# libxsmm/libxsmm

Measured on NVIDIA H100. Metric: batched BRGEMM GFLOP/s (bf16, m=n=k=64, br=8, batch=65536/GPU, unique operands), higher is better.
Workload: dtype bf16

## Files before the change

### libxsmm_b200/csrc/gemm_tc.cu

```cuda
#include <cuda.h>
#include <cuda_runtime.h>
#include <stdint.h>
#include <stdio.h>
#include <stdlib.h>
#include <string.h>
#include "xb_internal.h"
#include "xb_device.cuh"
#include "xb_tma.cuh"
#include "xb_wgmma.cuh"
#include "xb_epilogue.cuh"

namespace {

enum { XB_WG_SS16 = 0, XB_WG_RS16 = 1, XB_WG_RS8 = 2 };

struct WgParams {
  int m, n, k;
  int kchunks, kc_elems, kinst;
  int stages, stage_bytes, a_bytes, tx_bytes;
  int bf16;
  int sgn;
  unsigned long long br;
  long long count;
  char* c; long long tile_stride_c, ldc;
  int ep_mode, c_esz, beta0;
  float scf;
  const int4* sets; char* const* cptrs; int pair;
};

template <int NC>
__device__ __forceinline__ void wg_mma16(int bf16, float (&d)[NC / 2], uint64_t a, uint64_t b, int scale_d) {
  if (NC == 16) { if (bf16) xb_wgmma_ss_bf16_n16<1>(*reinterpret_cast<float(*)[8]>(&d), a, b, scale_d); else xb_wgmma_ss_f16_n16<1>(*reinterpret_cast<float(*)[8]>(&d), a, b, scale_d); }
  if (NC == 32) { if (bf16) xb_wgmma_ss_bf16_n32<1>(*reinterpret_cast<float(*)[16]>(&d), a, b, scale_d); else xb_wgmma_ss_f16_n32<1>(*reinterpret_cast<float(*)[16]>(&d), a, b, scale_d); }
  if (NC == 64) { if (bf16) xb_wgmma_ss_bf16_n64<1>(*reinterpret_cast<float(*)[32]>(&d), a, b, scale_d); else xb_wgmma_ss_f16_n64<1>(*reinterpret_cast<float(*)[32]>(&d), a, b, scale_d); }
}
template <int NC>
__device__ __forceinline__ void wg_mma16_rs(int bf16, float (&d)[NC / 2], const uint32_t (&a)[4], uint64_t b, int scale_d) {
  if (NC == 16) { if (bf16) xb_wgmma_rs_bf16_n16(*reinterpret_cast<float(*)[8]>(&d), a, b, scale_d); else xb_wgmma_rs_f16_n16(*reinterpret_cast<float(*)[8]>(&d), a, b, scale_d); }
  if (NC == 32) { if (bf16) xb_wgmma_rs_bf16_n32(*reinterpret_cast<float(*)[16]>(&d), a, b, scale_d); else xb_wgmma_rs_f16_n32(*reinterpret_cast<float(*)[16]>(&d), a, b, scale_d); }
  if (NC == 64) { if (bf16) xb_wgmma_rs_bf16_n64(*reinterpret_cast<float(*)[32]>(&d), a, b, scale_d); else xb_wgmma_rs_f16_n64(*reinterpret_cast<float(*)[32]>(&d), a, b, scale_d); }
}
#define XB_WG_I8(N) \
  switch (sgn) { case 0: xb_wgmma_rs_u8u8_n##N(*reinterpret_cast<int(*)[N / 2]>(&d), a, b, scale_d); break; \
                 case 1: xb_wgmma_rs_u8s8_n##N(*reinterpret_cast<int(*)[N / 2]>(&d), a, b, scale_d); break; \
                 case 2: xb_wgmma_rs_s8u8_n##N(*reinterpret_cast<int(*)[N / 2]>(&d), a, b, scale_d); break; \
                 default: xb_wgmma_rs_s8s8_n##N(*reinterpret_cast<int(*)[N / 2]>(&d), a, b, scale_d); break; }
template <int NC>
__device__ __forceinline__ void wg_mma8_rs(int sgn, float (&d)[NC / 2], const uint32_t (&a)[4], uint64_t b, int scale_d) {
  if (NC == 16) { XB_WG_I8(16) }
  if (NC == 32) { XB_WG_I8(32) }
  if (NC == 64) { XB_WG_I8(64) }
}
#undef XB_WG_I8

template <int AMODE, int NC, int NCH, int WG>
__global__ void __launch_bounds__(WG * 128 + 32, (NCH == 1 && WG == 1) ? 3 : 1)
gemm_wg_kernel(const __grid_constant__ CUtensorMap map_a, const __grid_constant__ CUtensorMap map_b, const WgParams P) {
  extern __shared__ uint8_t smem_raw[];
  uint8_t* smem = (uint8_t*)(((uintptr_t)smem_raw + 1023) & ~(uintptr_t)1023);
  const uint32_t smem_base = xb_smem_u32(smem);
  const int S = P.stages;
  const uint32_t full0 = xb_smem_u32(smem + (size_t)S * P.stage_bytes), empty0 = full0 + 8 * S;
  const int warp = threadIdx.x >> 5, lane = threadIdx.x & 31;
  const long long G = gridDim.x, b = blockIdx.x;
  const long long n_local = (b < P.count) ? (P.count - b + G - 1) / G : 0;
  const bool pooled = P.sets != nullptr;

  if (threadIdx.x == 0) {
    asm volatile("prefetch.tensormap [%0];" :: "l"(&map_a) : "memory");
    asm volatile("prefetch.tensormap [%0];" :: "l"(&map_b) : "memory");
    for (int i = 0; i < S; ++i) { xb_mbar_init(full0 + 8 * i, 1); xb_mbar_init(empty0 + 8 * i, 4 * WG); }
    asm volatile("fence.mbarrier_init.release.cluster;" ::: "memory");
  }
  __syncthreads();

  if (warp == 4 * WG) {
    if (lane == 0) {
      int stage = 0; uint32_t phase = 0;
      for (long long i = 0; i < n_local; ++i) {
        const long long t = b + i * G;
        int ta0 = (int)t, ta1 = (int)t, tb = (int)t, m1 = 64;
        if (pooled) {
          const int4 st = P.sets[t];
          ta0 = st.x; ta1 = P.pair ? st.y : st.x; tb = st.z; m1 = P.pair ? 0 : 64;
        }
        for (unsigned long long r = 0; r < P.br; ++r) {
          for (int kc = 0; kc < P.kchunks; ++kc) {
            xb_mbar_wait(empty0 + 8 * stage, phase ^ 1);
            const uint32_t full = full0 + 8 * stage, sa = smem_base + stage * P.stage_bytes, sb = sa + P.a_bytes;
            xb_mbar_expect_tx(full, (uint32_t)P.tx_bytes);
            if (AMODE == XB_WG_SS16) {
              xb_tma_load_4d(sa, &map_a, full, 0, kc * 64, (int)r, ta0);
              if (WG == 2) xb_tma_load_4d(sa + 8192, &map_a, full, m1, kc * 64, (int)r, ta1);
            } else {
              xb_tma_load_4d(sa, &map_a, full, 0, kc * 32, (int)r, ta0);
            }
            xb_tma_load_4d(sb, &map_b, full, kc * P.kc_elems, 0, (int)r, tb);
            if (++stage == S) { stage = 0; phase ^= 1; }
          }
        }
      }
    }
    return;
  }

  const int g = warp >> 2, wq = warp & 3;
  const int row_a = 64 * g + 16 * wq + (lane >> 2), q = lane & 3;
  const int loads = (int)P.br * P.kchunks;
  float acc[NCH][NC / 2];
  int stage = 0; uint32_t phase = 0;
  for (long long i = 0; i < n_local; ++i) {
    const long long t = b + i * G;
    int kc = 0, prev = -1;
    for (int l = 0; l < loads; ++l) {
      xb_mbar_wait(full0 + 8 * stage, phase);
      const uint32_t sa = smem_base + stage * P.stage_bytes, sb = sa + P.a_bytes;
      const int krem = P.k - kc * P.kc_elems;
      const int ksteps = (krem >= P.kc_elems) ? P.kc_elems / P.kinst : (krem + P.kinst - 1) / P.kinst;
      xb_wgmma_fence();
      for (int ks = 0; ks < ksteps; ++ks) {
        const int scale_d = (l > 0 || ks > 0) ? 1 : 0;
        if (AMODE == XB_WG_SS16) {
          const uint64_t ad = xb_wg_desc(sa + 8192u * g + 2048u * ks, 8192, 1024, 1);
#pragma unroll
          for (int c = 0; c < NCH; ++c) wg_mma16<NC>(P.bf16, acc[c], ad, xb_wg_desc(sb + (uint32_t)(c * NC * 128) + 32u * ks, 16, 1024, 1), scale_d);
        } else {
          const uint32_t* w = reinterpret_cast<const uint32_t*>(smem + (size_t)stage * P.stage_bytes);
          uint32_t a[4];
#pragma unroll
          for (int j = 0; j < 4; ++j) {
            const int rr = row_a + 8 * (j & 1), kw = 8 * ks + q + 4 * (j >> 1);
            a[j] = (rr < P.m) ? w[kw * P.m + rr] : 0u;
          }
#pragma unroll
          for (int c = 0; c < NCH; ++c) {
            const uint64_t bd = xb_wg_desc(sb + (uint32_t)(c * NC * 128) + 32u * ks, 16, 1024, 1);
            if (AMODE == XB_WG_RS16) wg_mma16_rs<NC>(P.bf16, acc[c], a, bd, scale_d);
            else wg_mma8_rs<NC>(P.sgn, acc[c], a, bd, scale_d);
          }
        }
      }
      xb_wgmma_commit();
      xb_wgmma_wait<1>();
      if (prev >= 0) { __syncwarp(); if (lane == 0) xb_mbar_arrive(empty0 + 8 * prev); }
      prev = stage;
      if (++kc == P.kchunks) kc = 0;
      if (++stage == S) { stage = 0; phase ^= 1; }
    }
    xb_wgmma_wait<0>();
    if (prev >= 0) { __syncwarp(); if (lane == 0) xb_mbar_arrive(empty0 + 8 * prev); }
    char* ctile; int row0 = 64 * g;
    if (!pooled) ctile = P.c + t * P.tile_stride_c;
    else if (P.pair) { ctile = P.cptrs[2 * t + g]; row0 = 0; }
    else ctile = P.cptrs[t];
    if (ctile == nullptr) continue;
    char* cbase = ctile - (long long)(64 * g - row0) * P.c_esz;
#pragma unroll
    for (int c = 0; c < NCH; ++c) {
      if (c * NC >= P.n) break;
      xb_ep_store_frag<NC / 2>(P.ep_mode, P.beta0, *reinterpret_cast<const uint32_t(*)[NC / 2]>(&acc[c]), cbase, 64 * g, c * NC,
                               P.m + (64 * g - row0), P.n, P.ldc * P.c_esz, P.c_esz, P.scf);
    }
  }
}

int g_num_sms = 0;

int env_int(const char* name, int fallback) {
  const char* e = getenv(name);
  return (e != nullptr && *e != 0) ? atoi(e) : fallback;
}

int num_sms() {
  if (g_num_sms == 0) {
    int dev = 0; cudaGetDevice(&dev);
    cudaDeviceGetAttribute(&g_num_sms, cudaDevAttrMultiProcessorCount, dev);
    if (g_num_sms <= 0) g_num_sms = 132;
  }
  return g_num_sms;
}

template <int AMODE, int NC, int NCH, int WG>
cudaError_t launch_one(long long grid, size_t smem, cudaStream_t stream, const CUtensorMap& ma, const CUtensorMap& mb, const WgParams& P) {
  static unsigned long long done = 0ull;
  if (xb_rt_first_use_on_device(&done)) cudaFuncSetAttribute(gemm_wg_kernel<AMODE, NC, NCH, WG>, cudaFuncAttributeMaxDynamicSharedMemorySize, 227 * 1024);
  gemm_wg_kernel<AMODE, NC, NCH, WG><<<(unsigned int)grid, WG * 128 + 32, smem, stream>>>(ma, mb, P);
  return cudaGetLastError();
}

template <int AMODE, int WG>
cudaError_t launch_n(int nt, long long grid, size_t smem, cudaStream_t stream, const CUtensorMap& ma, const CUtensorMap& mb, const WgParams& P) {
  switch (nt) {
    case 16:  return launch_one<AMODE, 16, 1, WG>(grid, smem, stream, ma, mb, P);
    case 32:  return launch_one<AMODE, 32, 1, WG>(grid, smem, stream, ma, mb, P);
    case 64:  return launch_one<AMODE, 64, 1, WG>(grid, smem, stream, ma, mb, P);
    case 128: return launch_one<AMODE, 64, 2, WG>(grid, smem, stream, ma, mb, P);
    default:  return launch_one<AMODE, 64, 4, WG>(grid, smem, stream, ma, mb, P);
  }
}

int n_tile(int n) { return n <= 16 ? 16 : (n <= 32 ? 32 : (n <= 64 ? 64 : (n <= 128 ? 128 : 256))); }

void plan_stages(WgParams& P, int nt, int wg, int* ctas) {
  int c = (nt == 64 && wg == 1) || nt < 64 ? 3 : 1;
  while (c > 1 && 2 * P.stage_bytes + 2048 > (227 * 1024) / c) --c;
  int st = ((227 * 1024) / c - 2048) / P.stage_bytes; if (st > 8) st = 8; if (st < 2) st = 2;
  P.stages = st; *ctas = c;
}

int wg_launch(int amode, int wg, int nt, const WgParams& P, int ctas, const CUtensorMap& ma, const CUtensorMap& mb, const char* where) {
  const size_t smem = (size_t)P.stages * P.stage_bytes + 1024  + 2 * 8 * P.stages;
  long long grid = P.count; if (grid > (long long)num_sms() * ctas) grid = (long long)num_sms() * ctas; if (grid < 1) grid = 1;
  cudaStream_t stream = (cudaStream_t)xb_rt_stream();
  cudaError_t e;
  if (amode == XB_WG_SS16) e = (wg == 2) ? launch_n<XB_WG_SS16, 2>(nt, grid, smem, stream, ma, mb, P) : launch_n<XB_WG_SS16, 1>(nt, grid, smem, stream, ma, mb, P);
  else if (amode == XB_WG_RS16) e = (wg == 2) ? launch_n<XB_WG_RS16, 2>(nt, grid, smem, stream, ma, mb, P) : launch_n<XB_WG_RS16, 1>(nt, grid, smem, stream, ma, mb, P);
  else e = (wg == 2) ? launch_n<XB_WG_RS8, 2>(nt, grid, smem, stream, ma, mb, P) : launch_n<XB_WG_RS8, 1>(nt, grid, smem, stream, ma, mb, P);
  xb_rt_count_launch();
  if (e != cudaSuccess) { xb_rt_note_error((int)e, where); return (int)e; }
  return 0;
}

}

extern "C" int xb_gemm_tc_supported(const xb_gemm_desc* d);
extern "C" int xb_gemm_tc_shape_ok(const xb_gemm_desc* d) {
  xb_gemm_desc t = *d;
  t.br_type = 0;
  return xb_gemm_tc_supported(&t);
}

extern "C" int xb_gemm_tc_supported(const xb_gemm_desc* d) {
  const unsigned int bad = LIBXSMM_GEMM_FLAG_TRANS_A | LIBXSMM_GEMM_FLAG_TRANS_B | LIBXSMM_GEMM_FLAG_VNNI_A
                         | LIBXSMM_GEMM_FLAG_VNNI_B | LIBXSMM_GEMM_FLAG_VNNI_C | LIBXSMM_GEMM_FLAG_DECOMPRESS_A_VIA_BITMASK;
  if ((d->flags & bad) != 0) return 0;
  if (!(d->ta == d->tb && (d->ta == LIBXSMM_DATATYPE_BF16 || d->ta == LIBXSMM_DATATYPE_F16))) return 0;
  if (d->tcomp != LIBXSMM_DATATYPE_F32) return 0;
  if (d->ta == LIBXSMM_DATATYPE_BF16 && !(d->tc == LIBXSMM_DATATYPE_F32 || d->tc == LIBXSMM_DATATYPE_BF16)) return 0;
  if (d->ta == LIBXSMM_DATATYPE_F16 && !(d->tc == LIBXSMM_DATATYPE_F32 || d->tc == LIBXSMM_DATATYPE_F16)) return 0;
  if (d->m < 16 || d->n < 16 || d->k < 16 || d->m > 128 || d->n > 256 || d->k > 4096) return 0;
  if ((d->lda % 8) != 0 || (d->ldb % 8) != 0) return 0;
  if (!(d->br_type == 0 || d->br_type == 3)) return 0;
  if (d->br_type == 3 && ((d->br_stride_a % 16) != 0 || (d->br_stride_b % 16) != 0 || d->br_stride_a <= 0 || d->br_stride_b <= 0)) return 0;
  return 1;
}

static int tc_launch_common(const xb_gemm_launch* L, const xb_tc_pool* pool);
extern "C" int xb_gemm_tc_launch(const xb_gemm_launch* L) { return tc_launch_common(L, nullptr); }
extern "C" int xb_gemm_tc_launch_pooled(const xb_gemm_desc* d, const xb_tc_pool* pool, unsigned long long br, long long count) {
  xb_gemm_launch L; memset(&L, 0, sizeof(L));
  L.d = *d; L.count = count; L.br = br;
  L.a = pool->base_a; L.b = pool->base_b; L.c = (void*)pool->cptrs;
  L.tile_stride_a = pool->set_a; L.tile_stride_b = pool->set_b; L.tile_stride_c = 16;
  return tc_launch_common(&L, pool);
}

static int tc_launch_common(const xb_gemm_launch* L, const xb_tc_pool* pool) {
  const xb_gemm_desc& d = L->d;
  const char* a = (const char*)L->a; const char* b = (const char*)L->b; char* c = (char*)L->c;
  long long sa = L->tile_stride_a, sb = L->tile_stride_b, sc = L->tile_stride_c;
  unsigned long long br = L->br;
  if (L->recs != nullptr) return xb_gemm_simt_launch(L);
  if (a == nullptr && c == nullptr) { a = (const char*)L->one.a; b = (const char*)L->one.b; c = (char*)L->one.c; br = L->one.br; sa = sb = sc = 0; }
  if (d.br_type == 0 && pool == nullptr) br = 1;
  const int es = 2;
  const bool aligned = (((uintptr_t)a | (uintptr_t)b) & 15) == 0 && (sa % 16) == 0 && (sb % 16) == 0
                    && (L->count == 1 || (sa > 0 && sb > 0));
  xb_encode_tiled_fn enc = xb_tma_encoder();
  if (br == 0 || !aligned || L->count <= 0 || br > 0x7fffffffull || L->count > 0x7fffffffll || enc == nullptr) {
    return (pool != nullptr) ? 1 : xb_gemm_simt_launch(L);
  }

  const int wg = (d.m <= 64 && !(pool != nullptr && pool->pair)) ? 1 : 2;
  const int nt = n_tile(d.n);
  WgParams P; memset(&P, 0, sizeof(P));
  P.m = d.m; P.n = d.n; P.k = d.k;
  P.kc_elems = 64; P.kinst = 16; P.kchunks = (d.k + 63) / 64;
  P.a_bytes = wg * 8192; P.stage_bytes = P.a_bytes + nt * 128; P.tx_bytes = P.stage_bytes;
  P.bf16 = (d.ta == LIBXSMM_DATATYPE_BF16) ? 1 : 0;
  P.br = br; P.count = L->count; P.c = c; P.tile_stride_c = sc; P.ldc = d.ldc;
  if (pool != nullptr) { P.sets = (const int4*)pool->sets; P.cptrs = (char* const*)pool->cptrs; P.pair = pool->pair; }
  P.beta0 = (d.flags & LIBXSMM_GEMM_FLAG_BETA_0) ? 1 : 0;
  P.ep_mode = xb_ep_mode(d.ta, d.tc, &P.c_esz);
  int ctas = 1;
  plan_stages(P, nt, wg, &ctas);

  const CUtensorMapDataType dt = P.bf16 ? CU_TENSOR_MAP_DATA_TYPE_BFLOAT16 : CU_TENSOR_MAP_DATA_TYPE_FLOAT16;
  const cuuint32_t estr[4] = {1, 1, 1, 1};
  const size_t ext_a = ((size_t)(d.k - 1) * d.lda + d.m) * es, ext_b = ((size_t)(d.n - 1) * d.ldb + d.k) * es;
  const cuuint64_t pad_a = (ext_a + 15) & ~(size_t)15, pad_b = (ext_b + 15) & ~(size_t)15;
  CUtensorMap map_a, map_b;
  {
    const cuuint64_t dims[4] = {(cuuint64_t)d.m, (cuuint64_t)d.k, (cuuint64_t)br, (cuuint64_t)(pool ? pool->nsets_a : L->count)};
    const cuuint64_t strides[3] = {(cuuint64_t)d.lda * es, pool ? (cuuint64_t)pool->blk_a : ((d.br_type == 3) ? (cuuint64_t)d.br_stride_a : pad_a),
                                   pool ? (cuuint64_t)pool->set_a : ((L->count > 1) ? (cuuint64_t)sa : pad_a)};
    const cuuint32_t box[4] = {64, 64, 1, 1};
    if (CUDA_SUCCESS != enc(&map_a, dt, 4, (void*)a, dims, strides, box, estr, CU_TENSOR_MAP_INTERLEAVE_NONE,
                            CU_TENSOR_MAP_SWIZZLE_128B, CU_TENSOR_MAP_L2_PROMOTION_L2_256B, CU_TENSOR_MAP_FLOAT_OOB_FILL_NONE))
      return (pool != nullptr) ? 1 : xb_gemm_simt_launch(L);
  }
  {
    const cuuint64_t dims[4] = {(cuuint64_t)d.k, (cuuint64_t)d.n, (cuuint64_t)br, (cuuint64_t)(pool ? pool->nsets_b : L->count)};
    const cuuint64_t strides[3] = {(cuuint64_t)d.ldb * es, pool ? (cuuint64_t)pool->blk_b : ((d.br_type == 3) ? (cuuint64_t)d.br_stride_b : pad_b),
                                   pool ? (cuuint64_t)pool->set_b : ((L->count > 1) ? (cuuint64_t)sb : pad_b)};
    const cuuint32_t box[4] = {64, (cuuint32_t)nt, 1, 1};
    if (CUDA_SUCCESS != enc(&map_b, dt, 4, (void*)b, dims, strides, box, estr, CU_TENSOR_MAP_INTERLEAVE_NONE,
                            CU_TENSOR_MAP_SWIZZLE_128B, CU_TENSOR_MAP_L2_PROMOTION_L2_256B, CU_TENSOR_MAP_FLOAT_OOB_FILL_NONE))
      return (pool != nullptr) ? 1 : xb_gemm_simt_launch(L);
  }
  return wg_launch(XB_WG_SS16, wg, nt, P, ctas, map_a, map_b, "gemm_tc");
}

extern "C" int xb_gemm_ts_supported(const xb_gemm_desc* d) {
  const unsigned int bad = LIBXSMM_GEMM_FLAG_TRANS_A | LIBXSMM_GEMM_FLAG_TRANS_B | LIBXSMM_GEMM_FLAG_VNNI_B | LIBXSMM_GEMM_FLAG_VNNI_C
                         | LIBXSMM_GEMM_FLAG_DECOMPRESS_A_VIA_BITMASK | LIBXSMM_GEMM_FLAG_INTLV_A_FORMAT;
  const int a8 = (d->ta == LIBXSMM_DATATYPE_I8 || d->ta == LIBXSMM_DATATYPE_U8), b8 = (d->tb == LIBXSMM_DATATYPE_I8 || d->tb == LIBXSMM_DATATYPE_U8);
  static int enabled = -1;
  if (enabled < 0) enabled = env_int("LIBXSMM_B200_TS", 1) != 0 ? 1 : 0;
  if (!enabled || (d->flags & bad) != 0 || d->fuse_colbias != 0 || d->cp_op != 0) return 0;
  if (a8 && b8) {
    if (d->tcomp != LIBXSMM_DATATYPE_I32 || !(d->tc == LIBXSMM_DATATYPE_I32 || d->tc == LIBXSMM_DATATYPE_F32)) return 0;
    if ((d->flags & LIBXSMM_GEMM_FLAG_VNNI_A) == 0 && d->tc != LIBXSMM_DATATYPE_F32) return 0;
    if ((d->k % 4) != 0 || (d->ldb % 16) != 0) return 0;
  } else if (d->ta == d->tb && (d->ta == LIBXSMM_DATATYPE_BF16 || d->ta == LIBXSMM_DATATYPE_F16)) {
    if ((d->flags & LIBXSMM_GEMM_FLAG_VNNI_A) == 0 || d->tcomp != LIBXSMM_DATATYPE_F32) return 0;
    if (d->ta == LIBXSMM_DATATYPE_BF16 && !(d->tc == LIBXSMM_DATATYPE_F32 || d->tc == LIBXSMM_DATATYPE_BF16)) return 0;
    if (d->ta == LIBXSMM_DATATYPE_F16 && !(d->tc == LIBXSMM_DATATYPE_F32 || d->tc == LIBXSMM_DATATYPE_F16)) return 0;
    if ((d->k % 2) != 0 || (d->ldb % 8) != 0) return 0;
  } else return 0;
  if (d->m < 4 || d->m > 128 || (d->m % 4) != 0 || (d->lda % 4) != 0 || d->n < 1 || d->n > 128 || d->k > 8192) return 0;
  if (!(d->br_type == 0 || d->br_type == 3)) return 0;
  if (d->br_type == 3 && ((d->br_stride_a % 16) != 0 || (d->br_stride_b % 16) != 0 || d->br_stride_a <= 0 || d->br_stride_b <= 0)) return 0;
  return 1;
}

extern "C" int xb_gemm_ts_launch(const xb_gemm_launch* L) {
  const xb_gemm_desc& d = L->d;
  const char* a = (const char*)L->a; const char* b = (const char*)L->b; char* c = (char*)L->c;
  long long sa = L->tile_stride_a, sb = L->tile_stride_b, sc = L->tile_stride_c;
  unsigned long long br = L->br;
  if (L->recs != nullptr) return xb_gemm_simt_launch(L);
  if (a == nullptr && c == nullptr) { a = (const char*)L->one.a; b = (const char*)L->one.b; c = (char*)L->one.c; br = L->one.br; sa = sb = sc = 0; }
  if (d.br_type == 0) br = 1;
  const bool aligned = (((uintptr_t)a | (uintptr_t)b) & 15) == 0 && (sa % 16) == 0 && (sb % 16) == 0 && (L->count == 1 || (sa > 0 && sb > 0));
  xb_encode_tiled_fn enc = xb_tma_encoder();
  if (br == 0 || !aligned || L->count <= 0 || br > 0x7fffffffull || L->count > 0x7fffffffll || enc == nullptr) return xb_gemm_simt_launch(L);

  const int is_i8 = (d.ta == LIBXSMM_DATATYPE_I8 || d.ta == LIBXSMM_DATATYPE_U8);
  const int v = is_i8 ? 4 : 2, es = is_i8 ? 1 : 2;
  const int wg = (d.m <= 64) ? 1 : 2, nt = n_tile(d.n);
  WgParams P; memset(&P, 0, sizeof(P));
  P.m = d.m; P.n = d.n; P.k = d.k;
  P.kc_elems = 128 / es; P.kinst = is_i8 ? 32 : 16; P.kchunks = (d.k + P.kc_elems - 1) / P.kc_elems;
  P.a_bytes = (d.m * 128 + 1023) & ~1023;
  P.stage_bytes = P.a_bytes + nt * 128; P.tx_bytes = d.m * 128 + nt * 128;
  P.bf16 = (d.ta == LIBXSMM_DATATYPE_BF16) ? 1 : 0;
  P.sgn = ((d.ta == LIBXSMM_DATATYPE_I8) ? 2 : 0) | ((d.tb == LIBXSMM_DATATYPE_I8) ? 1 : 0);
  P.br = br; P.count = L->count; P.c = c; P.tile_stride_c = sc; P.ldc = d.ldc;
  P.beta0 = (d.flags & LIBXSMM_GEMM_FLAG_BETA_0) ? 1 : 0; P.scf = L->one.scf;
  P.ep_mode = xb_ep_mode(d.ta, d.tc, &P.c_esz);
  int ctas = 1;
  plan_stages(P, nt, wg, &ctas);

  const cuuint32_t estr[4] = {1, 1, 1, 1};
  const size_t ext_a = ((size_t)(d.k / v - 1) * d.lda + d.m) * 4, ext_b = ((size_t)(d.n - 1) * d.ldb + d.k) * es;
  const cuuint64_t pad_a = (ext_a + 15) & ~(size_t)15, pad_b = (ext_b + 15) & ~(size_t)15;
  CUtensorMap map_a, map_b;
  {
    const cuuint64_t dims[4] = {(cuuint64_t)d.m, (cuuint64_t)(d.k / v), (cuuint64_t)br, (cuuint64_t)L->count};
    const cuuint64_t strides[3] = {(cuuint64_t)d.lda * 4, (d.br_type == 3) ? (cuuint64_t)d.br_stride_a : pad_a, (L->count > 1) ? (cuuint64_t)sa : pad_a};
    const cuuint32_t box[4] = {(cuuint32_t)d.m, 32, 1, 1};
    if (CUDA_SUCCESS != enc(&map_a, CU_TENSOR_MAP_DATA_TYPE_UINT32, 4, (void*)a, dims, strides, box, estr, CU_TENSOR_MAP_INTERLEAVE_NONE,
                            CU_TENSOR_MAP_SWIZZLE_NONE, CU_TENSOR_MAP_L2_PROMOTION_L2_256B, CU_TENSOR_MAP_FLOAT_OOB_FILL_NONE)) return xb_gemm_simt_launch(L);
  }
  {
    const CUtensorMapDataType dt = is_i8 ? CU_TENSOR_MAP_DATA_TYPE_UINT8 : (P.bf16 ? CU_TENSOR_MAP_DATA_TYPE_BFLOAT16 : CU_TENSOR_MAP_DATA_TYPE_FLOAT16);
    const cuuint64_t dims[4] = {(cuuint64_t)d.k, (cuuint64_t)d.n, (cuuint64_t)br, (cuuint64_t)L->count};
    const cuuint64_t strides[3] = {(cuuint64_t)d.ldb * es, (d.br_type == 3) ? (cuuint64_t)d.br_stride_b : pad_b, (L->count > 1) ? (cuuint64_t)sb : pad_b};
    const cuuint32_t box[4] = {(cuuint32_t)P.kc_elems, (cuuint32_t)nt, 1, 1};
    if (CUDA_SUCCESS != enc(&map_b, dt, 4, (void*)b, dims, strides, box, estr, CU_TENSOR_MAP_INTERLEAVE_NONE,
                            CU_TENSOR_MAP_SWIZZLE_128B, CU_TENSOR_MAP_L2_PROMOTION_L2_256B, CU_TENSOR_MAP_FLOAT_OOB_FILL_NONE)) return xb_gemm_simt_launch(L);
  }
  return wg_launch(is_i8 ? XB_WG_RS8 : XB_WG_RS16, wg, nt, P, ctas, map_a, map_b, "gemm_ts");
}
```

Before: 87740.

## Skip reloading smem-resident operand tiles for pooled BRGEMM and template k-steps

For pooled launches whose whole reduction fits in the stage ring, the stage count is rounded to a multiple of the per-task load count. The producer then skips TMA loads of A/B tiles that match the task held in the same slots, arriving on the barrier directly when nothing needs loading. Pooled tasks are also given contiguous ranges per CTA so that consecutive tasks are more likely to share operands. Separately, the per-chunk k-step count becomes a template parameter, so the wgmma loop is fully unrolled and the runtime krem arithmetic goes away. This adds more kernel instantiations, and for a partial last k-chunk it always runs four steps, relying on TMA zero fill.

```diff
diff --git a/libxsmm_b200/csrc/gemm_tc.cu b/libxsmm_b200/csrc/gemm_tc.cu
--- a/libxsmm_b200/csrc/gemm_tc.cu
+++ b/libxsmm_b200/csrc/gemm_tc.cu
@@ -17,7 +17,9 @@
 struct WgParams {
   int m, n, k;
   int kchunks, kc_elems, kinst;
+  int ksteps;
   int stages, stage_bytes, a_bytes, tx_bytes;
+  int resident;
   int bf16;
   int sgn;
   unsigned long long br;
@@ -53,7 +55,7 @@
 }
 #undef XB_WG_I8
 
-template <int AMODE, int NC, int NCH, int WG>
+template <int AMODE, int NC, int NCH, int WG, int KS>
 __global__ void __launch_bounds__(WG * 128 + 32, (NCH == 1 && WG == 1) ? 3 : 1)
 gemm_wg_kernel(const __grid_constant__ CUtensorMap map_a, const __grid_constant__ CUtensorMap map_b, const WgParams P) {
   extern __shared__ uint8_t smem_raw[];
@@ -63,8 +65,9 @@
   const uint32_t full0 = xb_smem_u32(smem + (size_t)S * P.stage_bytes), empty0 = full0 + 8 * S;
   const int warp = threadIdx.x >> 5, lane = threadIdx.x & 31;
   const long long G = gridDim.x, b = blockIdx.x;
-  const long long n_local = (b < P.count) ? (P.count - b + G - 1) / G : 0;
   const bool pooled = P.sets != nullptr;
+  const long long first = pooled ? P.count * b / G : b;
+  const long long n_local = pooled ? P.count * (b + 1) / G - first : ((b < P.count) ? (P.count - b + G - 1) / G : 0);
 
   if (threadIdx.x == 0) {
     asm volatile("prefetch.tensormap [%0];" :: "l"(&map_a) : "memory");
@@ -78,24 +81,35 @@
     if (lane == 0) {
       int stage = 0; uint32_t phase = 0;
       for (long long i = 0; i < n_local; ++i) {
-        const long long t = b + i * G;
+        const long long t = pooled ? first + i : b + i * G;
         int ta0 = (int)t, ta1 = (int)t, tb = (int)t, m1 = 64;
+        bool ld_a0 = true, ld_a1 = (WG == 2), ld_b = true;
         if (pooled) {
           const int4 st = P.sets[t];
           ta0 = st.x; ta1 = P.pair ? st.y : st.x; tb = st.z; m1 = P.pair ? 0 : 64;
+          if (AMODE == XB_WG_SS16 && P.resident > 0 && i >= P.resident) {
+            const int4 held = P.sets[t - P.resident];
+            ld_a0 = ta0 != held.x; ld_a1 = ld_a1 && ta1 != (P.pair ? held.y : held.x); ld_b = tb != held.z;
+          }
         }
+        const uint32_t tx = (AMODE == XB_WG_SS16) ? (ld_a0 ? 8192u : 0u) + (ld_a1 ? 8192u : 0u) + (ld_b ? (uint32_t)(P.stage_bytes - P.a_bytes) : 0u)
+                                                  : (uint32_t)P.tx_bytes;
         for (unsigned long long r = 0; r < P.br; ++r) {
           for (int kc = 0; kc < P.kchunks; ++kc) {
             xb_mbar_wait(empty0 + 8 * stage, phase ^ 1);
             const uint32_t full = full0 + 8 * stage, sa = smem_base + stage * P.stage_bytes, sb = sa + P.a_bytes;
-            xb_mbar_expect_tx(full, (uint32_t)P.tx_bytes);
-            if (AMODE == XB_WG_SS16) {
-              xb_tma_load_4d(sa, &map_a, full, 0, kc * 64, (int)r, ta0);
-              if (WG == 2) xb_tma_load_4d(sa + 8192, &map_a, full, m1, kc * 64, (int)r, ta1);
+            if (tx == 0) {
+              xb_mbar_arrive(full);
             } else {
-              xb_tma_load_4d(sa, &map_a, full, 0, kc * 32, (int)r, ta0);
+              xb_mbar_expect_tx(full, tx);
+              if (AMODE == XB_WG_SS16) {
+                if (ld_a0) xb_tma_load_4d(sa, &map_a, full, 0, kc * 64, (int)r, ta0);
+                if (ld_a1) xb_tma_load_4d(sa + 8192, &map_a, full, m1, kc * 64, (int)r, ta1);
+              } else {
+                xb_tma_load_4d(sa, &map_a, full, 0, kc * 32, (int)r, ta0);
+              }
+              if (ld_b) xb_tma_load_4d(sb, &map_b, full, kc * P.kc_elems, 0, (int)r, tb);
             }
-            xb_tma_load_4d(sb, &map_b, full, kc * P.kc_elems, 0, (int)r, tb);
             if (++stage == S) { stage = 0; phase ^= 1; }
           }
         }
@@ -110,15 +124,14 @@
   float acc[NCH][NC / 2];
   int stage = 0; uint32_t phase = 0;
   for (long long i = 0; i < n_local; ++i) {
-    const long long t = b + i * G;
-    int kc = 0, prev = -1;
+    const long long t = pooled ? first + i : b + i * G;
+    int prev = -1;
     for (int l = 0; l < loads; ++l) {
       xb_mbar_wait(full0 + 8 * stage, phase);
       const uint32_t sa = smem_base + stage * P.stage_bytes, sb = sa + P.a_bytes;
-      const int krem = P.k - kc * P.kc_elems;
-      const int ksteps = (krem >= P.kc_elems) ? P.kc_elems / P.kinst : (krem + P.kinst - 1) / P.kinst;
       xb_wgmma_fence();
-      for (int ks = 0; ks < ksteps; ++ks) {
+#pragma unroll
+      for (int ks = 0; ks < KS; ++ks) {
         const int scale_d = (l > 0 || ks > 0) ? 1 : 0;
         if (AMODE == XB_WG_SS16) {
           const uint64_t ad = xb_wg_desc(sa + 8192u * g + 2048u * ks, 8192, 1024, 1);
@@ -144,7 +157,6 @@
       xb_wgmma_wait<1>();
       if (prev >= 0) { __syncwarp(); if (lane == 0) xb_mbar_arrive(empty0 + 8 * prev); }
       prev = stage;
-      if (++kc == P.kchunks) kc = 0;
       if (++stage == S) { stage = 0; phase ^= 1; }
     }
     xb_wgmma_wait<0>();
@@ -180,22 +192,31 @@
   return g_num_sms;
 }
 
-template <int AMODE, int NC, int NCH, int WG>
+template <int AMODE, int NC, int NCH, int WG, int KS>
 cudaError_t launch_one(long long grid, size_t smem, cudaStream_t stream, const CUtensorMap& ma, const CUtensorMap& mb, const WgParams& P) {
   static unsigned long long done = 0ull;
-  if (xb_rt_first_use_on_device(&done)) cudaFuncSetAttribute(gemm_wg_kernel<AMODE, NC, NCH, WG>, cudaFuncAttributeMaxDynamicSharedMemorySize, 227 * 1024);
-  gemm_wg_kernel<AMODE, NC, NCH, WG><<<(unsigned int)grid, WG * 128 + 32, smem, stream>>>(ma, mb, P);
+  if (xb_rt_first_use_on_device(&done)) cudaFuncSetAttribute(gemm_wg_kernel<AMODE, NC, NCH, WG, KS>, cudaFuncAttributeMaxDynamicSharedMemorySize, 227 * 1024);
+  gemm_wg_kernel<AMODE, NC, NCH, WG, KS><<<(unsigned int)grid, WG * 128 + 32, smem, stream>>>(ma, mb, P);
   return cudaGetLastError();
+}
+
+template <int AMODE, int NC, int NCH, int WG>
+cudaError_t launch_k(long long grid, size_t smem, cudaStream_t stream, const CUtensorMap& ma, const CUtensorMap& mb, const WgParams& P) {
+  if constexpr (NCH == 1) {
+    if (P.ksteps == 1) return launch_one<AMODE, NC, NCH, WG, 1>(grid, smem, stream, ma, mb, P);
+    if (P.ksteps == 2) return launch_one<AMODE, NC, NCH, WG, 2>(grid, smem, stream, ma, mb, P);
+  }
+  return launch_one<AMODE, NC, NCH, WG, 4>(grid, smem, stream, ma, mb, P);
 }
 
 template <int AMODE, int WG>
 cudaError_t launch_n(int nt, long long grid, size_t smem, cudaStream_t stream, const CUtensorMap& ma, const CUtensorMap& mb, const WgParams& P) {
   switch (nt) {
-    case 16:  return launch_one<AMODE, 16, 1, WG>(grid, smem, stream, ma, mb, P);
-    case 32:  return launch_one<AMODE, 32, 1, WG>(grid, smem, stream, ma, mb, P);
-    case 64:  return launch_one<AMODE, 64, 1, WG>(grid, smem, stream, ma, mb, P);
-    case 128: return launch_one<AMODE, 64, 2, WG>(grid, smem, stream, ma, mb, P);
-    default:  return launch_one<AMODE, 64, 4, WG>(grid, smem, stream, ma, mb, P);
+    case 16:  return launch_k<AMODE, 16, 1, WG>(grid, smem, stream, ma, mb, P);
+    case 32:  return launch_k<AMODE, 32, 1, WG>(grid, smem, stream, ma, mb, P);
+    case 64:  return launch_k<AMODE, 64, 1, WG>(grid, smem, stream, ma, mb, P);
+    case 128: return launch_k<AMODE, 64, 2, WG>(grid, smem, stream, ma, mb, P);
+    default:  return launch_k<AMODE, 64, 4, WG>(grid, smem, stream, ma, mb, P);
   }
 }
 
@@ -206,6 +227,8 @@
   while (c > 1 && 2 * P.stage_bytes + 2048 > (227 * 1024) / c) --c;
   int st = ((227 * 1024) / c - 2048) / P.stage_bytes; if (st > 8) st = 8; if (st < 2) st = 2;
   P.stages = st; *ctas = c;
+  const int need = (P.k + P.kinst - 1) / P.kinst;
+  P.ksteps = (P.kchunks == 1 && need <= 2) ? need : 4;
 }
 
 int wg_launch(int amode, int wg, int nt, const WgParams& P, int ctas, const CUtensorMap& ma, const CUtensorMap& mb, const char* where) {
@@ -284,6 +307,10 @@
   P.ep_mode = xb_ep_mode(d.ta, d.tc, &P.c_esz);
   int ctas = 1;
   plan_stages(P, nt, wg, &ctas);
+  if (pool != nullptr && br * (unsigned long long)P.kchunks <= (unsigned long long)P.stages) {
+    const int loads = (int)br * P.kchunks;
+    P.resident = P.stages / loads; P.stages = P.resident * loads;
+  }
 
   const CUtensorMapDataType dt = P.bf16 ? CU_TENSOR_MAP_DATA_TYPE_BFLOAT16 : CU_TENSOR_MAP_DATA_TYPE_FLOAT16;
   const cuuint32_t estr[4] = {1, 1, 1, 1};
```

Result: no change. 87970 (median of 6 runs) (+0.3%).
